# ziyu0425/PDE-Solver

Hardware: NVIDIA B200
Metric: GDOF/s (higher is better)
Workload: dtype f64

## Files before the change

### pde_solver_b200/csrc/heat2.cu

```cuda
#include <cuda.h>

#include <cmath>

#include "device.cuh"
#include "tma.cuh"

namespace {

#ifndef H_RR_STAGES
#define H_RR_STAGES 3
#endif
template <bool RR>
struct HS { static constexpr int N = RR ? H_RR_STAGES : 4; };

template <int CW, int YSB>
struct HG {
  static constexpr int TX = CW - 2, YSA = YSB + 1, TY = 2 * YSB, RA = TY + 2;
  static constexpr int BX = TX + 4, BYX = TY + 4, BYB = TY + 2;
  static constexpr int XBOX = BX * BYX, BBOX = BX * BYB;
  static constexpr int XS = (XBOX + 15) / 16 * 16, BS = (BBOX + 15) / 16 * 16;
  static constexpr int STAGE = XS + BS;
  static constexpr int RING = RA * CW;
  static constexpr int NT = 2 * CW;
  static constexpr size_t smem(int nst) { return ((size_t)nst * STAGE + 4 * RING) * sizeof(double) + nst * sizeof(uint64_t); }
};

struct H2Coef {
  double c0, cxp, cxm, cyp, cym, czp, czm, cxyp, cxym, cxzp, cxzm, cyzp, cyzm, cdp, cdm;
};
struct H2Args {
  double* y;
  double a0, a1, k1;
  int do_reduce;
  double* yc;
  int cnn0, cnn1, cnzl, cz0, cPX;
  long long cplane;
};
struct H2Geom {
  int nn0, nn1, nzl, z0, nzg, PX;
  long long plane;
  int ntx, nty, nzc, zc;
};

template <int YS>
__device__ __forceinline__ void h2_contrib(const H2Coef& C, const double (&V)[YS + 2][3], double (&aP)[YS], double (&a0)[YS],
                                           double (&aM)[YS]) {
#pragma unroll
  for (int j = 0; j < YS; ++j) {
    const int r = j + 1;
    double t = fma(C.c0, V[r][1], a0[j]);
    t = fma(C.cxp, V[r][2], t);
    t = fma(C.cxm, V[r][0], t);
    t = fma(C.cyp, V[r + 1][1], t);
    t = fma(C.cym, V[r - 1][1], t);
    t = fma(C.cxyp, V[r + 1][2], t);
    a0[j] = fma(C.cxym, V[r - 1][0], t);
    double p = fma(C.czp, V[r][1], aP[j]);
    p = fma(C.cxzp, V[r][2], p);
    p = fma(C.cyzp, V[r + 1][1], p);
    aP[j] = fma(C.cdp, V[r + 1][2], p);
    double m = C.czm * V[r][1];
    m = fma(C.cxzm, V[r][0], m);
    m = fma(C.cyzm, V[r - 1][1], m);
    aM[j] = fma(C.cdm, V[r - 1][0], m);
  }
}

template <int CW, int YSB, bool RR>
__global__ void __launch_bounds__(2 * CW, CW == 64 ? ((RR && H_RR_STAGES == 3) ? 4 : (YSB >= 4 ? 3 : (YSB == 3 ? 4 : 5))) : 6)
k_heat_post2(const __grid_constant__ CUtensorMap tmx, const __grid_constant__ CUtensorMap tmb,
             const __grid_constant__ H2Coef C, const __grid_constant__ H2Args a, const __grid_constant__ H2Geom ge,
             ReduceBuf red, double* red_out) {
  using G = HG<CW, YSB>;
  constexpr int YSA = G::YSA;
  constexpr int H_STAGES = HS<RR>::N;
  extern __shared__ __align__(128) unsigned char smem_raw[];
  double* const stage0 = reinterpret_cast<double*>(smem_raw);
  double* const ring0 = stage0 + H_STAGES * G::STAGE;
  uint64_t* const bars = reinterpret_cast<uint64_t*>(ring0 + 4 * G::RING);

  const int t = threadIdx.x;
  const int item = blockIdx.x;
  const int itx = item % ge.ntx;
  const int ity = (item / ge.ntx) % ge.nty;
  const int izc = item / (ge.ntx * ge.nty);
  const int x0 = itx * G::TX, y0 = ity * G::TY;
  const int za = izc * ge.zc;
  const int zb = min(za + ge.zc, ge.nzl);
  const int nplanes = zb - za + 4;
  const uint32_t bar0 = smem_u32(bars);
  const uint32_t stg0 = smem_u32(stage0);
  constexpr uint32_t STAGE_BYTES = G::STAGE * 8;

  auto issue = [&](int n) {
    const uint32_t bar = bar0 + 8 * (n % H_STAGES);
    const uint32_t dst = stg0 + (n % H_STAGES) * STAGE_BYTES;
    mbar_expect_tx(bar, (uint32_t)((G::XBOX + (n >= 2 ? G::BBOX : 0)) * 8));
    tma_load_4d(dst, &tmx, x0 - 2, y0 - 2, za - 2 + n + PDE_NG, 0, bar);
    if (n >= 2) tma_load_4d(dst + G::XS * 8, &tmb, x0 - 2, y0 - 1, za - 3 + n + PDE_NG, 0, bar);
  };
  if (t == 0) {
#pragma unroll
    for (int s = 0; s < H_STAGES; ++s) mbar_init(bar0 + 8 * s, 1);
    asm volatile("fence.mbarrier_init.release.cluster;" ::: "memory");
  }
  __syncthreads();
  if (t == 0)
    for (int n = 0; n < 2 && n < nplanes; ++n) issue(n);

  const int c = t % CW;
  const int s = t / CW;
  const int ix = x0 - 1 + c;
  const int cB = min(max(c, 1), CW - 2);
  const bool xfree = ix >= 1 && ix <= ge.nn0 - 2;
  unsigned mAb = 0, mBb = 0, okB = 0;
#pragma unroll
  for (int j = 0; j < YSA; ++j) {
    const int iy = y0 - 1 + s * YSA + j;
    if (xfree && iy >= 1 && iy <= ge.nn1 - 2) mAb |= 1u << j;
  }
#pragma unroll
  for (int j = 0; j < YSB; ++j) {
    const int iy = y0 + s * YSB + j;
    const bool in = c >= 1 && c <= G::TX && ix < ge.nn0 && iy < ge.nn1;
    if (in) okB |= 1u << j;
    if (in && xfree && iy >= 1 && iy <= ge.nn1 - 2) mBb |= 1u << j;
  }
  const int offA = (s * YSA) * G::BX + c;
  const int offbA = G::XS + (s * YSA) * G::BX + c + 1;
  const int offbB = G::XS + (s * YSB + 1) * G::BX + cB + 1;
  const int offxB = (s * YSB + 2) * G::BX + cB + 1;
  const int ringA = (s * YSA) * CW + c;
  const int ringB = (s * YSB) * CW + cB - 1;
  double* yrun = a.y + ((long long)ge.PX * (y0 + s * YSB) + ix) + ge.plane * za;

  double aA[YSA], aB[YSA], aC[YSA];
  double bA_[YSB], bB_[YSB], bC_[YSB];
#pragma unroll
  for (int j = 0; j < YSA; ++j) aA[j] = aB[j] = aC[j] = 0.0;
#pragma unroll
  for (int j = 0; j < YSB; ++j) bA_[j] = bB_[j] = bC_[j] = 0.0;
  double red_by = 0.0;

  auto body = [&](int i, double (&aP)[YSA], double (&a0)[YSA], double (&aM)[YSA], double (&bP)[YSB], double (&b0)[YSB],
                  double (&bM)[YSB]) {
    const int stage = i % H_STAGES;
    const int q = za - 2 + i;
    const int pA = q - 1;
    const int pB = q - 2;
    const bool finA = i >= 2, finB = i >= 4;
    double xB0[YSB], bvB[YSB];
    if (!RR && finB) {
      const double* const sx2 = stage0 + ((i - 2) % H_STAGES) * G::STAGE + offxB;
      const double* const sb1 = stage0 + ((i - 1) % H_STAGES) * G::STAGE + offbB;
#pragma unroll
      for (int j = 0; j < YSB; ++j) { xB0[j] = sx2[j * G::BX]; bvB[j] = sb1[j * G::BX]; }
    }
    mbar_wait(bar0 + 8 * stage, (uint32_t)((i / H_STAGES) & 1));
    const double* const sx = stage0 + stage * G::STAGE;
    {
      double V[YSA + 2][3];
      const double* const sp = sx + offA;
#pragma unroll
      for (int r = 0; r < YSA + 2; ++r)
#pragma unroll
        for (int cc = 0; cc < 3; ++cc)
          V[r][cc] = ((r == 0 && cc == 2) || (r == YSA + 1 && cc == 0)) ? 0.0 : sp[r * G::BX + cc];
      h2_contrib<YSA>(C, V, aP, a0, aM);
    }
    if (finA) {
      const int gz = pA + ge.z0;
      const bool zfree = gz >= 1 && gz <= ge.nzg - 2;
      const unsigned mA = zfree ? mAb : 0u;
      double* const ds = ring0 + ((pA + 4) & 3) * G::RING + ringA;
      const double* const sb = sx + offbA;
#pragma unroll
      for (int j = 0; j < YSA; ++j) ds[j * CW] = ((mA >> j) & 1u) ? a.a0 * (sb[j * G::BX] - aP[j]) : 0.0;
    }
    __syncthreads();
    if (t == 0 && i + 2 < nplanes) issue(i + 2);
    if (!RR && finA) {
      double V[YSB + 2][3];
      const double* const rp = ring0 + ((pA + 4) & 3) * G::RING + ringB;
#pragma unroll
      for (int r = 0; r < YSB + 2; ++r)
#pragma unroll
        for (int cc = 0; cc < 3; ++cc)
          V[r][cc] = ((r == 0 && cc == 2) || (r == YSB + 1 && cc == 0)) ? 0.0 : rp[r * CW + cc];
      h2_contrib<YSB>(C, V, bP, b0, bM);
    }
    if (RR && finB) {
      const int gz = pB + ge.z0;
      const int Z = (gz >> 1) - a.cz0;
      constexpr int NCX = G::TX / 2, NCY = G::TY / 2;
      if (!(gz & 1) && Z >= 0 && Z < a.cnzl && t < NCX * NCY) {
        const int cx = t % NCX, cy = t / NCX;
        const int X = (x0 >> 1) + cx, Y = (y0 >> 1) + cy;
        if (X < a.cnn0 && Y < a.cnn1) {
          const int o = (1 + 2 * cy) * CW + 1 + 2 * cx;
          const double* const r0 = ring0 + ((pB + 4) & 3) * G::RING + o;
          const double* const rm = ring0 + ((pB + 3) & 3) * G::RING + o;
          const double* const rp = ring0 + ((pB + 5) & 3) * G::RING + o;
          const double nb = ((r0[1] + r0[-1]) + (r0[CW] + r0[-CW])) + ((r0[CW + 1] + r0[-CW - 1]) + (rp[0] + rm[0])) +
                            ((rp[1] + rm[-1]) + (rp[CW] + rm[-CW])) + (rp[CW + 1] + rm[-CW - 1]);
          const int cgz = gz >> 1;
          const bool cfree = X >= 1 && X <= a.cnn0 - 2 && Y >= 1 && Y <= a.cnn1 - 2 && cgz >= 1 && cgz <= (ge.nzg >> 1) - 1;
          a.yc[(long long)a.cPX * Y + a.cplane * Z + X] = cfree ? fma(0.5, nb, r0[0]) : 0.0;
        }
      }
    }
    if (!RR && finB) {
      const int gz = pB + ge.z0;
      const bool zfree = gz >= 1 && gz <= ge.nzg - 2;
      const unsigned mB = zfree ? mBb : 0u;
      const double* const dso = ring0 + ((pB + 4) & 3) * G::RING + ringB + CW + 1;
#pragma unroll
      for (int j = 0; j < YSB; ++j) {
        const bool m = (mB >> j) & 1u;
        const double x2 = m ? fma(a.k1, dso[j * CW], fma(-a.a1, bP[j], xB0[j])) : xB0[j];
        if ((okB >> j) & 1u) yrun[j * (long long)ge.PX] = x2;
        red_by = fma(m ? bvB[j] : 0.0, x2, red_by);
      }
      yrun += ge.plane;
    }
  };

  for (int i = 0; i < nplanes; i += 3) {
    body(i, aA, aB, aC, bB_, bC_, bA_);
    if (i + 1 < nplanes) body(i + 1, aB, aC, aA, bC_, bA_, bB_);
    if (i + 2 < nplanes) body(i + 2, aC, aA, aB, bA_, bB_, bC_);
  }
  if (a.do_reduce) {
    double v[1] = {red_by};
    block_reduce_finalize<1>(v, red, red_out);
  }
}

template <int CW, int YSB, bool RR>
int launch_t(pde_ctx* c, const Grid& g, const OpDev& op, const double* x0, const double* b, const H2Args& ha_in) {
  using G = HG<CW, YSB>;
  H2Geom ge;
  ge.nn0 = g.nn[0]; ge.nn1 = g.nn[1]; ge.nzl = g.nzl; ge.z0 = g.z0; ge.nzg = g.nzg; ge.PX = g.PX; ge.plane = g.plane;
  ge.ntx = (g.nn[0] + G::TX - 1) / G::TX;
  ge.nty = (g.nn[1] + G::TY - 1) / G::TY;
  static const int zc_env = env_int("PDE_B200_P2_ZC", 64);
  int zc = zc_env < 4 ? 4 : zc_env;
  while (zc > 8 && (long long)ge.ntx * ge.nty * ((g.nzl + zc - 1) / zc) < 6LL * c->sm_count) zc /= 2;
  ge.nzc = (g.nzl + zc - 1) / zc;
  ge.zc = (g.nzl + ge.nzc - 1) / ge.nzc;
  ge.nzc = (g.nzl + ge.zc - 1) / ge.zc;
  const long long items = (long long)ge.ntx * ge.nty * ge.nzc;
  if (items > RED_MAX_BLOCKS) return 2;
  auto kern = k_heat_post2<CW, YSB, RR>;
  static bool attr_set = false;
  if (!attr_set) {
    CUDA_OK(cudaFuncSetAttribute(kern, cudaFuncAttributeMaxDynamicSharedMemorySize, (int)G::smem(HS<RR>::N)));
    CUDA_OK(cudaFuncSetAttribute(kern, cudaFuncAttributePreferredSharedMemoryCarveout, 100));
    attr_set = true;
  }
  CUtensorMap tmx, tmb;
  PDE_OK(field_tensor_map(x0, g, 1, G::BX, G::BYX, &tmx));
  PDE_OK(field_tensor_map(b, g, 1, G::BX, G::BYB, &tmb));
  H2Coef C;
  const double* h = op.h_int;
  C.c0 = h[0]; C.cxp = h[1]; C.cxm = h[2]; C.cyp = h[3]; C.cym = h[4]; C.czp = h[5]; C.czm = h[6]; C.cxyp = h[7];
  C.cxym = h[8]; C.cxzp = h[9]; C.cxzm = h[10]; C.cyzp = h[11]; C.cyzm = h[12]; C.cdp = h[13]; C.cdm = h[14];
  kern<<<(unsigned)items, G::NT, G::smem(HS<RR>::N), c->stream>>>(tmx, tmb, C, ha_in, ge, c->red, ha_in.do_reduce ? c->scal + ha_in.do_reduce - 1 : nullptr);
  c->launches++;
  CUDA_OK(cudaGetLastError());
  return 0;
}

bool heat2_applicable(const Grid& g, const OpDev& op) {
  static const int off = env_int("PDE_B200_NO_HEAT2", 0);
  if (off) return false;
  if (g.dim != 3 || g.nk != PDE_NOFF || op.ncomp != 1 || !op.uniform_diag) return false;
  return g.nn[0] >= 32 && g.nn[1] >= 8 && g.nzl >= 8;
}

template <bool RR>
int dispatch(pde_ctx* c, const Grid& g, const OpDev& op, const double* x0, const double* b, const H2Args& ha) {
  static const int cw_env = env_int("PDE_B200_P2_CW", 0);
  static const int ysb = env_int("PDE_B200_P2_YSB", 4);
  const int cw = cw_env ? cw_env : (g.nn[0] >= 128 ? 64 : 32);
  if (cw == 64 && ysb == 3) return launch_t<64, 3, RR>(c, g, op, x0, b, ha);
  if (cw == 64) return launch_t<64, 4, RR>(c, g, op, x0, b, ha);
  return launch_t<32, 4, RR>(c, g, op, x0, b, ha);
}

}

bool post2_applicable(const Grid& g, const OpDev& op) {
  if (g.dim != 3 || g.nk != PDE_NOFF || op.ncomp != 1 || !op.uniform_diag) return false;
  if (g.nn[0] < 32 || g.nn[1] < 8 || g.nzl < 8) return false;
  return !env_int("PDE_B200_NO_HEAT2", 0) || !env_int("PDE_B200_NO_POST2", 0);
}

int launch_heat_post2(pde_ctx* c, const Grid& g, const OpDev& op, const double* x0, const double* b, double* y, double c2_0,
                      double c1_1, double c2_1, int dot_slot, bool* handled) {
  *handled = false;
  if (!heat2_applicable(g, op) || !(c2_0 * op.h_dinv_int[0] > 0.0)) return 0;
  H2Args ha{};
  ha.y = y;
  ha.a0 = c2_0 * op.h_dinv_int[0];
  ha.a1 = c2_1 * op.h_dinv_int[0];
  ha.k1 = 1.0 + c1_1 + ha.a1 / ha.a0;
  ha.do_reduce = dot_slot >= 0 ? dot_slot + 1 : 0;
  const int rc = dispatch<false>(c, g, op, x0, b, ha);
  if (rc == 0) *handled = true;
  return rc == 2 ? 0 : rc;
}

int launch_heat_resid_restrict(pde_ctx* c, const Grid& gf, const Grid& gc, const OpDev& op, const double* x, const double* b,
                               double* bcoarse, bool* handled) {
  *handled = false;
  static const int off = env_int("PDE_B200_NO_RR", 0);
  if (off || !heat2_applicable(gf, op)) return 0;
  if (gf.nc[0] != 2 * gc.nc[0] || gf.nc[1] != 2 * gc.nc[1] || gf.nc[2] != 2 * gc.nc[2] || gf.z0 != 2 * gc.z0) return 0;
  H2Args ha{};
  ha.a0 = 1.0;
  ha.yc = bcoarse;
  ha.cnn0 = gc.nn[0]; ha.cnn1 = gc.nn[1]; ha.cnzl = gc.nzl; ha.cz0 = gc.z0; ha.cPX = gc.PX; ha.cplane = gc.plane;
  const int rc = dispatch<true>(c, gf, op, x, b, ha);
  if (rc == 0) *handled = true;
  return rc == 2 ? 0 : rc;
}
```

### pde_solver_b200/csrc/kernels.cu

```cuda
#include <cstring>

#include "device.cuh"
#include "tma.cuh"

template <int NC>
struct IntCoef {
  double c[PDE_NOFF][NC * NC];
};

struct StencilDev {
  const double* x;
  const double* b;
  double* y;
  const double* xprev;
  int prev_mode;
  double bconst[3];
  double bscale, ascale, c1, c2, s0;
  int do_reduce;
  int first2;
  double* defer;
};

template <int NC, bool CHEBY>
__global__ void __launch_bounds__(128)
// ... 616 lines not shown
    return 0;
  }
#define FACE_LAUNCH(CH, FU)                                                                                      \
  DISPATCH_NC(op.ncomp, (k_face_rows<NC, CH, FU><<<blocks, FACE_NT, 0, c->stream>>>(g, bc, fs, op.coef, op.dinv, op.load, \
                                                                               sd, c->red, out)))
  if (a.cheby) {
    if (full) { FACE_LAUNCH(true, true); } else { FACE_LAUNCH(true, false); }
  } else {
    if (full) { FACE_LAUNCH(false, true); } else { FACE_LAUNCH(false, false); }
  }
#undef FACE_LAUNCH
  c->launches++;
  CUDA_OK(cudaGetLastError());
  return 0;
}

__global__ void __launch_bounds__(256)
k_cg_update_flat(double* __restrict__ x, double* __restrict__ r, const double* __restrict__ p,
                 const double* __restrict__ q, long long n, int ncomp, long long cs, const double* __restrict__ scal,
                 int s_rho, int s_pap, ReduceBuf red, double* out_rho_new) {
  const double pap = scal[s_pap], rho = scal[s_rho];
  const double alpha = pap > 0.0 ? rho / pap : 0.0;
  const long long n2 = n >> 1;
  double rr = 0.0;
  for (int cidx = 0; cidx < ncomp; ++cidx) {
    double2* x2 = reinterpret_cast<double2*>(x + cidx * cs);
    double2* r2 = reinterpret_cast<double2*>(r + cidx * cs);
    const double2* p2 = reinterpret_cast<const double2*>(p + cidx * cs);
    const double2* q2 = reinterpret_cast<const double2*>(q + cidx * cs);
    if (x == nullptr) {
      for (long long i = (long long)blockIdx.x * blockDim.x + threadIdx.x; i < n2; i += (long long)gridDim.x * blockDim.x) {
        const double2 qv = q2[i];
        double2 rv = r2[i];
        rv.x = fma(-alpha, qv.x, rv.x);
        rv.y = fma(-alpha, qv.y, rv.y);
        r2[i] = rv;
        rr = fma(rv.x, rv.x, rr);
        rr = fma(rv.y, rv.y, rr);
      }
      continue;
    }
    for (long long i = (long long)blockIdx.x * blockDim.x + threadIdx.x; i < n2; i += (long long)gridDim.x * blockDim.x) {
      const double2 pv = p2[i], qv = q2[i];
      double2 xv = x2[i], rv = r2[i];
      xv.x = fma(alpha, pv.x, xv.x);
      xv.y = fma(alpha, pv.y, xv.y);
      rv.x = fma(-alpha, qv.x, rv.x);
      rv.y = fma(-alpha, qv.y, rv.y);
      x2[i] = xv;
      r2[i] = rv;
      rr = fma(rv.x, rv.x, rr);
      rr = fma(rv.y, rv.y, rr);
    }
  }
  double v[2] = {0.0, rr};
  block_reduce_finalize<2>(v, red, out_rho_new);
}

__global__ void __launch_bounds__(256)
k_cg_pupdate_flat(double* __restrict__ p, const double* __restrict__ z, long long n, int ncomp, long long cs,
                  const double* __restrict__ scal, int s_rho, int s_rho_new, int first, double* __restrict__ x,
                  int s_pap) {
  double beta = 0.0;
  if (!first) {
    const double rho = scal[s_rho];
    beta = rho > 0.0 ? scal[s_rho_new] / rho : 0.0;
  }
  const long long n2 = n >> 1;
  if (x != nullptr && !first) {
    const double pap = scal[s_pap], rho = scal[s_rho];
    const double alpha = pap > 0.0 ? rho / pap : 0.0;
    for (int cidx = 0; cidx < ncomp; ++cidx) {
      double2* p2 = reinterpret_cast<double2*>(p + cidx * cs);
      double2* x2 = reinterpret_cast<double2*>(x + cidx * cs);
      const double2* z2 = reinterpret_cast<const double2*>(z + cidx * cs);
      for (long long i = (long long)blockIdx.x * blockDim.x + threadIdx.x; i < n2; i += (long long)gridDim.x * blockDim.x) {
        const double2 zv = z2[i];
        double2 pv = p2[i], xv = x2[i];
        xv.x = fma(alpha, pv.x, xv.x);
        xv.y = fma(alpha, pv.y, xv.y);
        pv.x = fma(beta, pv.x, zv.x);
        pv.y = fma(beta, pv.y, zv.y);
        x2[i] = xv;
        p2[i] = pv;
      }
    }
    return;
  }
  for (int cidx = 0; cidx < ncomp; ++cidx) {
    double2* p2 = reinterpret_cast<double2*>(p + cidx * cs);
    const double2* z2 = reinterpret_cast<const double2*>(z + cidx * cs);
    for (long long i = (long long)blockIdx.x * blockDim.x + threadIdx.x; i < n2; i += (long long)gridDim.x * blockDim.x) {
      const double2 zv = z2[i];
      double2 pv = first ? make_double2(0.0, 0.0) : p2[i];
      pv.x = fma(beta, pv.x, zv.x);
      pv.y = fma(beta, pv.y, zv.y);
      p2[i] = pv;
    }
  }
}

int launch_cg_update(pde_ctx* c, const Grid& g, const OpDev& op, double* x, double* r, const double* p,
                     const double* q, int slot_rho, int slot_pap, int slot_rho_new, int slot_rr, int jacobi) {
  if (slot_rr != slot_rho_new + 1) PDE_FAIL("cg_update needs adjacent (rho_new, rr) slots");
  if (!jacobi) {
    int blocks = flat_blocks(c, g.total / 2, 256 * 2);
    k_cg_update_flat<<<blocks, 256, 0, c->stream>>>(x, r, p, q, g.total, op.ncomp, g.comp_stride, c->scal, slot_rho,
                                                    slot_pap, c->red, c->scal + slot_rho_new);
    c->launches++;
    CUDA_OK(cudaGetLastError());
    return 0;
  }
  RowLaunch rl = row_launch(c, g);
  DISPATCH_NC(op.ncomp, (k_cg_update<NC><<<rl.grid, rl.block, 0, c->stream>>>(
                            g, op.dinv, x, r, p, q, c->scal, slot_rho, slot_pap, c->red, c->scal + slot_rho_new,
                            c->scal + slot_rr)));
  c->launches++;
  CUDA_OK(cudaGetLastError());
  return 0;
}

int launch_cg_pupdate(pde_ctx* c, const Grid& g, const OpDev& op, double* p, const double* r_or_z, int slot_rho,
                      int slot_rho_new, int first, int jacobi, double* x_deferred, int slot_pap) {
  if (!jacobi) {
    int blocks = flat_blocks(c, g.total / 2, 256 * 2);
    k_cg_pupdate_flat<<<blocks, 256, 0, c->stream>>>(p, r_or_z, g.total, op.ncomp, g.comp_stride, c->scal, slot_rho,
                                                     slot_rho_new, first, x_deferred, slot_pap);
    c->launches++;
    CUDA_OK(cudaGetLastError());
    return 0;
  }
  RowLaunch rl = row_launch(c, g);
  DISPATCH_NC(op.ncomp, (k_cg_pupdate<NC><<<rl.grid, rl.block, 0, c->stream>>>(
                            g, op.dinv, p, r_or_z, c->scal, slot_rho, slot_rho_new, first, jacobi)));
  c->launches++;
  CUDA_OK(cudaGetLastError());
  return 0;
}

__global__ void __launch_bounds__(256)
k_dot(const double* __restrict__ a, const double* __restrict__ b, long long n, int ncomp, long long cs,
      ReduceBuf red, double* out) {
  double s = 0.0;
  const long long n2 = n >> 1;
  for (int cidx = 0; cidx < ncomp; ++cidx) {
    const double2* a2 = reinterpret_cast<const double2*>(a + cidx * cs);
    const double2* b2 = reinterpret_cast<const double2*>(b + cidx * cs);
    for (long long i = (long long)blockIdx.x * blockDim.x + threadIdx.x; i < n2; i += (long long)gridDim.x * blockDim.x) {
      const double2 u = a2[i], w = b2[i];
      s = fma(u.x, w.x, s);
      s = fma(u.y, w.y, s);
    }
  }
  double v[1] = {s};
  block_reduce_finalize<1>(v, red, out);
}

__global__ void __launch_bounds__(256)
k_axpy(double* __restrict__ y, const double* __restrict__ x, double alpha, long long n, int ncomp, long long cs,
       int mode) {
  const long long n2 = n >> 1;
  for (int cidx = 0; cidx < ncomp; ++cidx) {
    double2* y2 = reinterpret_cast<double2*>(y + cidx * cs);
    const double2* x2 = reinterpret_cast<const double2*>(x + cidx * cs);
    for (long long i = (long long)blockIdx.x * blockDim.x + threadIdx.x; i < n2; i += (long long)gridDim.x * blockDim.x) {
      if (mode == 0) {
        double2 u = y2[i];
        const double2 w = x2[i];
        u.x = fma(alpha, w.x, u.x);
        u.y = fma(alpha, w.y, u.y);
        y2[i] = u;
      } else if (mode == 1) {
        y2[i] = x2[i];
      } else {
        y2[i] = make_double2(0.0, 0.0);
      }
    }
  }
}

__global__ void __launch_bounds__(256)
k_extrapolate(double* __restrict__ u, double* __restrict__ uold, double* __restrict__ e, long long n, int ncomp,
              long long cs) {
  const long long n2 = n >> 1;
  for (int cidx = 0; cidx < ncomp; ++cidx) {
    double2* u2 = reinterpret_cast<double2*>(u + cidx * cs);
    double2* o2 = reinterpret_cast<double2*>(uold + cidx * cs);
    double2* e2 = reinterpret_cast<double2*>(e + cidx * cs);
    for (long long i = (long long)blockIdx.x * blockDim.x + threadIdx.x; i < n2; i += (long long)gridDim.x * blockDim.x) {
      const double2 a = u2[i], b = o2[i];
      const double2 d = make_double2(a.x - b.x, a.y - b.y);
      e2[i] = d;
      o2[i] = a;
      u2[i] = make_double2(a.x + d.x, a.y + d.y);
    }
  }
}
int launch_extrapolate(pde_ctx* c, const Grid& g, int ncomp, double* u, double* uold, double* e) {
  int blocks = flat_blocks(c, g.total / 2, 256 * 4);
  k_extrapolate<<<blocks, 256, 0, c->stream>>>(u, uold, e, g.total, ncomp, g.comp_stride);
  c->launches++;
  CUDA_OK(cudaGetLastError());
  return 0;
}

int launch_dot(pde_ctx* c, const Grid& g, int ncomp, const double* a, const double* b, int slot) {
  int blocks = flat_blocks(c, g.total / 2, 256 * 4);
  k_dot<<<blocks, 256, 0, c->stream>>>(a, b, g.total, ncomp, g.comp_stride, c->red, c->scal + slot);
  c->launches++;
  CUDA_OK(cudaGetLastError());
  return 0;
}
static int launch_axpy_mode(pde_ctx* c, const Grid& g, int ncomp, double* y, const double* x, double alpha, int mode) {
  int blocks = flat_blocks(c, g.total / 2, 256 * 4);
  k_axpy<<<blocks, 256, 0, c->stream>>>(y, x, alpha, g.total, ncomp, g.comp_stride, mode);
  c->launches++;
  CUDA_OK(cudaGetLastError());
  return 0;
}
int launch_zero(pde_ctx* c, const Grid& g, int ncomp, double* a) { return launch_axpy_mode(c, g, ncomp, a, a, 0.0, 2); }
int launch_copy(pde_ctx* c, const Grid& g, int ncomp, double* dst, const double* src) {
  return launch_axpy_mode(c, g, ncomp, dst, src, 0.0, 1);
}
int launch_axpy(pde_ctx* c, const Grid& g, int ncomp, double* y, const double* x, double alpha) {
  return launch_axpy_mode(c, g, ncomp, y, x, alpha, 0);
}

template <int NC>
__global__ void __launch_bounds__(128)
k_cheby_first(const __grid_constant__ Grid g, const __grid_constant__ BcDev bc, const double* __restrict__ dinv,
              const double* b, double* x, double s) {
  const long long rows = (long long)g.nn[1] * g.nzl;
  for (long long row = (long long)blockIdx.x * blockDim.y + threadIdx.y; row < rows;
       row += (long long)gridDim.x * blockDim.y) {
    const int iy = (int)(row % g.nn[1]);
    const int lz = (int)(row / g.nn[1]);
    const int gz = lz + g.z0;
    const long long rbase = (long long)g.PX * iy + g.plane * lz;
    for (int ix = threadIdx.x; ix < g.nn[0]; ix += blockDim.x) {
      double bcv;
      const bool isdir = bc_node(g, bc, ix, iy, gz, &bcv);
      const int cls = node_class(g, ix, iy, gz);
#pragma unroll
      for (int i = 0; i < NC; ++i) {
        const long long ii = rbase + ix + i * g.comp_stride;
        x[ii] = isdir ? 0.0 : s * __ldg(dinv + cls * NC + i) * b[ii];
      }
    }
  }
}

int launch_cheby_first(pde_ctx* c, const Grid& g, const BcDev& bc, const OpDev& op, const double* b, double* x,
                       double s) {
  RowLaunch rl = row_launch(c, g);
  DISPATCH_NC(op.ncomp, (k_cheby_first<NC><<<rl.grid, rl.block, 0, c->stream>>>(g, bc, op.dinv, b, x, s)));
  c->launches++;
  CUDA_OK(cudaGetLastError());
  return 0;
}

template <int NC>
__global__ void __launch_bounds__(256)
k_restrict(const __grid_constant__ Grid gf, const __grid_constant__ Grid gc, const __grid_constant__ BcDev bcc,
           const double* __restrict__ rf, double* __restrict__ bc_out) {
  const unsigned n0 = (unsigned)gc.nn[0], n1 = (unsigned)gc.nn[1];
  const long long total = (long long)n0 * n1 * gc.nzl;
  const bool small = total < (1LL << 32);
  for (long long t = (long long)blockIdx.x * blockDim.x + threadIdx.x; t < total; t += (long long)gridDim.x * blockDim.x) {
    const unsigned row = small ? (unsigned)t / n0 : (unsigned)(t / n0);
    const int ix = (int)(t - (long long)row * n0);
    const int iy = (int)(row % n1);
    const int lz = (int)(row / n1);
    const int gz = lz + gc.z0;
    const long long cbase = (long long)gc.PX * iy + gc.plane * lz;
    const int fy = gf.nc[1] > 0 ? 2 * iy : 0;
    const int flz = (gf.nc[2] > 0 ? 2 * gz : 0) - gf.z0;
    const long long fi = (long long)gf.PX * fy + gf.plane * flz + 2 * ix;
    double bcv;
    const bool isdir = bc_node(gc, bcc, ix, iy, gz, &bcv);
#pragma unroll
    for (int i = 0; i < NC; ++i) {
      double s = 0.0;
      if (!isdir) {
        const double* rp = rf + i * gf.comp_stride;
        double nb = 0.0;
        for (int k = 1; k < gf.nk; ++k) nb += rp[fi + gf.koff[k]];
        s = rp[fi] + 0.5 * nb;
      }
      bc_out[cbase + ix + i * gc.comp_stride] = s;
    }
  }
}

int launch_restrict(pde_ctx* c, const Grid& gf, const Grid& gc, const BcDev& bcc, int ncomp, const double* rf,
                    double* bcoarse) {
  const int blocks = flat_blocks(c, (long long)gc.nn[0] * gc.nn[1] * gc.nzl, 256);
  DISPATCH_NC(ncomp, (k_restrict<NC><<<blocks, 256, 0, c->stream>>>(gf, gc, bcc, rf, bcoarse)));
  c->launches++;
  CUDA_OK(cudaGetLastError());
  return 0;
}

template <int NC>
__global__ void __launch_bounds__(256)
k_prolong_add(const __grid_constant__ Grid gf, const __grid_constant__ Grid gc, const __grid_constant__ BcDev bcf,
              const double* __restrict__ xc, double* __restrict__ xf, int ghost) {
  const int nzr = gf.nzl + 2 * ghost;
  const unsigned npair = (unsigned)(gf.nn[0] + 1) / 2;
  const long long total = (long long)gf.nn[1] * nzr * npair;
  const bool small = total < (1LL << 32);
  for (long long t = (long long)blockIdx.x * blockDim.x + threadIdx.x; t < total; t += (long long)gridDim.x * blockDim.x) {
    const unsigned row = small ? (unsigned)t / npair : (unsigned)(t / npair);
    const int k = (int)(t - (long long)row * npair);
    const int iy = (int)(row % (unsigned)gf.nn[1]);
    const int lz = (int)(row / (unsigned)gf.nn[1]) - ghost;
    const int gz = lz + gf.z0;
    if (gz < 0 || gz > gf.nzg - 1) continue;
    const int ix = 2 * k;
    double bcv;
    const bool f0 = !bc_node(gf, bcf, ix, iy, gz, &bcv);
    const bool f1 = ix + 1 < gf.nn[0] && !bc_node(gf, bcf, ix + 1, iy, gz, &bcv);
    if (!f0 && !f1) continue;
    const long long fbase = (long long)gf.PX * iy + gf.plane * lz;
    const int py = gf.nc[1] > 0 ? (iy & 1) : 0;
    const int pz = gf.nc[2] > 0 ? (gz & 1) : 0;
    const int cy = gf.nc[1] > 0 ? (iy - py) / 2 : 0;
    const int clz = (gf.nc[2] > 0 ? (gz - pz) / 2 : 0) - gc.z0;
    const long long lo = (long long)gc.PX * cy + gc.plane * clz + k;
    const long long cpy = (long long)gc.PX * py + gc.plane * pz;
#pragma unroll
    for (int i = 0; i < NC; ++i) {
      const double* cp = xc + i * gc.comp_stride;
      double2* fp = reinterpret_cast<double2*>(xf + fbase + ix + i * gf.comp_stride);
      double2 v = *fp;
      const double c0 = cp[lo];
      if (f0) v.x += 0.5 * (c0 + cp[lo + cpy]);
      if (f1) v.y += 0.5 * (c0 + cp[lo + 1 + cpy]);
      *fp = v;
    }
  }
}

int launch_prolong_add(pde_ctx* c, const Grid& gf, const Grid& gc, const BcDev& bcf, int ncomp, const double* xc,
                       double* xf, int ghost) {
  const long long total = (long long)gf.nn[1] * (gf.nzl + 2 * ghost) * ((gf.nn[0] + 1) / 2);
  if (gf.nn[1] * (long long)(gf.nzl + 2 * ghost) >= (1LL << 32)) PDE_FAIL("prolongation: too many rows");
  const int blocks = flat_blocks(c, total, 256);
  DISPATCH_NC(ncomp, (k_prolong_add<NC><<<blocks, 256, 0, c->stream>>>(gf, gc, bcf, xc, xf, ghost)));
  c->launches++;
  CUDA_OK(cudaGetLastError());
  return 0;
}

__global__ void __launch_bounds__(256)
k_dense_solve(int n, const double* __restrict__ Ainv, const long long* __restrict__ idx, const double* __restrict__ b,
              double* __restrict__ x) {
  const int warp = (blockIdx.x * blockDim.x + threadIdx.x) >> 5, lane = threadIdx.x & 31;
  if (warp >= n) return;
  double s = 0.0;
  for (int j = lane; j < n; j += 32) s = fma(Ainv[(size_t)warp * n + j], b[idx[j]], s);
#pragma unroll
  for (int o = 16; o > 0; o >>= 1) s += __shfl_down_sync(0xffffffffu, s, o);
  if (lane == 0) x[idx[warp]] = s;
}

int launch_dense_solve(pde_ctx* c, int n, const double* Ainv, const long long* idx, const double* b, double* x) {
  if (n <= 0) return 0;
  int blocks = (n * 32 + 255) / 256;
  k_dense_solve<<<blocks, 256, 0, c->stream>>>(n, Ainv, idx, b, x);
  c->launches++;
  CUDA_OK(cudaGetLastError());
  return 0;
}

__global__ void __launch_bounds__(256)
k_dense_gather(int n, const long long* __restrict__ idx, const double* __restrict__ b, double* __restrict__ bglob) {
  const int j = blockIdx.x * blockDim.x + threadIdx.x;
  if (j < n) bglob[j] = idx[j] >= 0 ? b[idx[j]] : 0.0;
}
__global__ void __launch_bounds__(256)
k_dense_solve_owned(int n, const double* __restrict__ Ainv, const long long* __restrict__ idx,
                    const double* __restrict__ bglob, double* __restrict__ x) {
  const int warp = (blockIdx.x * blockDim.x + threadIdx.x) >> 5, lane = threadIdx.x & 31;
  if (warp >= n || idx[warp] < 0) return;
  double s = 0.0;
  for (int j = lane; j < n; j += 32) s = fma(Ainv[(size_t)warp * n + j], bglob[j], s);
#pragma unroll
  for (int o = 16; o > 0; o >>= 1) s += __shfl_down_sync(0xffffffffu, s, o);
  if (lane == 0) x[idx[warp]] = s;
}
int launch_dense_gather(pde_ctx* c, int n, const long long* idx, const double* b, double* bglob) {
  if (n <= 0) return 0;
  k_dense_gather<<<(n + 255) / 256, 256, 0, c->stream>>>(n, idx, b, bglob);
  c->launches++;
  CUDA_OK(cudaGetLastError());
  return 0;
}
int launch_dense_solve_owned(pde_ctx* c, int n, const double* Ainv, const long long* idx, const double* bglob,
                             double* x) {
  if (n <= 0) return 0;
  k_dense_solve_owned<<<(n * 32 + 255) / 256, 256, 0, c->stream>>>(n, Ainv, idx, bglob, x);
  c->launches++;
  CUDA_OK(cudaGetLastError());
  return 0;
}

__global__ void __launch_bounds__(128)
k_fill_ic(const __grid_constant__ Grid g, const __grid_constant__ BcDev bc, double* __restrict__ u, double value,
          int fill, int apply_bc) {
  const long long rows = (long long)g.nn[1] * g.nzl;
  for (long long row = (long long)blockIdx.x * blockDim.y + threadIdx.y; row < rows;
       row += (long long)gridDim.x * blockDim.y) {
    const int iy = (int)(row % g.nn[1]);
    const int lz = (int)(row / g.nn[1]);
    const long long rbase = (long long)g.PX * iy + g.plane * lz;
    for (int ix = threadIdx.x; ix < g.nn[0]; ix += blockDim.x) {
      double bcv;
      const bool isdir = apply_bc && bc_node(g, bc, ix, iy, lz + g.z0, &bcv);
      if (isdir) u[rbase + ix] = bcv;
      else if (fill) u[rbase + ix] = value;
    }
  }
}
__global__ void __launch_bounds__(128)
k_fill_pattern(const __grid_constant__ Grid g, const __grid_constant__ BcDev bc, int ncomp, double* __restrict__ x) {
  const long long rows = (long long)g.nn[1] * g.nzl;
  for (long long row = (long long)blockIdx.x * blockDim.y + threadIdx.y; row < rows;
       row += (long long)gridDim.x * blockDim.y) {
    const int iy = (int)(row % g.nn[1]);
    const int lz = (int)(row / g.nn[1]);
    for (int ix = threadIdx.x; ix < g.nn[0]; ix += blockDim.x) {
      double bcv;
      const bool isdir = bc_node(g, bc, ix, iy, lz + g.z0, &bcv);
      const long long node = ((long long)(lz + g.z0) * g.nn[1] + iy) * g.nn[0] + ix;
      for (int i = 0; i < ncomp; ++i)
        x[(long long)g.PX * iy + g.plane * lz + ix + i * g.comp_stride] =
            isdir ? 0.0 : sin(0.37 * (double)(node % 1000003) + i) + 0.5;
    }
  }
}
int launch_fill_pattern(pde_ctx* c, const Grid& g, const BcDev& bc, int ncomp, double* x) {
  RowLaunch rl = row_launch(c, g);
  k_fill_pattern<<<rl.grid, rl.block, 0, c->stream>>>(g, bc, ncomp, x);
  c->launches++;
  CUDA_OK(cudaGetLastError());
  return 0;
}

__global__ void __launch_bounds__(128)
k_halo_verify(const __grid_constant__ Grid g, int ncomp, int depth, const double* __restrict__ x, double scale,
              unsigned long long* bad) {
  const long long rows = (long long)g.nn[1] * 2 * depth;
  unsigned long long nbad = 0;
  for (long long row = (long long)blockIdx.x * blockDim.y + threadIdx.y; row < rows;
       row += (long long)gridDim.x * blockDim.y) {
    const int iy = (int)(row % g.nn[1]);
    const int q = (int)(row / g.nn[1]);
    const int lz = q < depth ? -1 - q : g.nzl + (q - depth);
    const int gz = lz + g.z0;
    if (gz < 0 || gz > g.nzg - 1) continue;
    for (int ix = threadIdx.x; ix < g.nn[0]; ix += blockDim.x) {
      const long long node = ((long long)gz * g.nn[1] + iy) * g.nn[0] + ix;
      for (int i = 0; i < ncomp; ++i) {
        const double want = scale * (sin(0.37 * (double)(node % 1000003) + i) + 0.5);
        if (x[(long long)g.PX * iy + g.plane * lz + ix + i * g.comp_stride] != want) ++nbad;
      }
    }
  }
  if (nbad) atomicAdd(bad, nbad);
}
int launch_halo_verify(pde_ctx* c, const Grid& g, int ncomp, int depth, const double* x, double scale,
                       unsigned long long* bad) {
  RowLaunch rl = row_launch(c, g);
  k_halo_verify<<<rl.grid, rl.block, 0, c->stream>>>(g, ncomp, depth, x, scale, bad);
  c->launches++;
  CUDA_OK(cudaGetLastError());
  return 0;
}

int launch_fill_ic(pde_ctx* c, const Grid& g, const BcDev& bc, double* u, double value, int apply_bc) {
  RowLaunch rl = row_launch(c, g);
  k_fill_ic<<<rl.grid, rl.block, 0, c->stream>>>(g, bc, u, value, 1, apply_bc);
  c->launches++;
  CUDA_OK(cudaGetLastError());
  return 0;
}
int launch_apply_bc_values(pde_ctx* c, const Grid& g, const BcDev& bc, double* u) {
  RowLaunch rl = row_launch(c, g);
  k_fill_ic<<<rl.grid, rl.block, 0, c->stream>>>(g, bc, u, 0.0, 0, 1);
  c->launches++;
  CUDA_OK(cudaGetLastError());
  return 0;
}

template <bool PACK>
__global__ void __launch_bounds__(128)
k_pack(const __grid_constant__ Grid g, int ncomp, double* __restrict__ padded, double* __restrict__ dense,
       int interleave) {
  const long long rows = (long long)g.nn[1] * g.nzl;
  const long long nloc = (long long)g.nn[0] * rows;
  for (long long row = (long long)blockIdx.x * blockDim.y + threadIdx.y; row < rows;
       row += (long long)gridDim.x * blockDim.y) {
    const int iy = (int)(row % g.nn[1]);
    const int lz = (int)(row / g.nn[1]);
    const long long rbase = (long long)g.PX * iy + g.plane * lz;
    for (int ix = threadIdx.x; ix < g.nn[0]; ix += blockDim.x) {
      const long long node = row * g.nn[0] + ix;
      for (int i = 0; i < ncomp; ++i) {
        const long long di = interleave ? node * ncomp + i : i * nloc + node;
        if (PACK) dense[di] = padded[rbase + ix + i * g.comp_stride];
        else padded[rbase + ix + i * g.comp_stride] = dense[di];
      }
    }
  }
}
int launch_pack(pde_ctx* c, const Grid& g, int ncomp, const double* padded, double* dense, int interleave) {
  RowLaunch rl = row_launch(c, g);
  k_pack<true><<<rl.grid, rl.block, 0, c->stream>>>(g, ncomp, const_cast<double*>(padded), dense, interleave);
  c->launches++;
  CUDA_OK(cudaGetLastError());
  return 0;
}
int launch_unpack(pde_ctx* c, const Grid& g, int ncomp, const double* dense, double* padded, int interleave) {
  RowLaunch rl = row_launch(c, g);
  k_pack<false><<<rl.grid, rl.block, 0, c->stream>>>(g, ncomp, padded, const_cast<double*>(dense), interleave);
  c->launches++;
  CUDA_OK(cudaGetLastError());
  return 0;
}

template <int NC>
__global__ void __launch_bounds__(128)
k_cell_rhs(const __grid_constant__ Grid g, const __grid_constant__ SimplexGeom sg, const double* __restrict__ u,
           double* __restrict__ rhs, int mode, double lam, double mu, double Emod) {
  const int axm[3] = {0, g.dim == 2 ? 2 : 1, 2};
  const long long rows = (long long)g.nn[1] * g.nzl;
  const double w = sg.vol / (double)(g.dim + 1);
  for (long long row = (long long)blockIdx.x * blockDim.y + threadIdx.y; row < rows;
       row += (long long)gridDim.x * blockDim.y) {
    const int iy = (int)(row % g.nn[1]);
    const int lz = (int)(row / g.nn[1]);
    const int gz = lz + g.z0;
    const long long rbase = (long long)g.PX * iy + g.plane * lz;
    for (int ix = threadIdx.x; ix < g.nn[0]; ix += blockDim.x) {
      const long long idx = rbase + ix;
      double acc = 0.0;
      for (int o = 0; o < 8; ++o) {
        const int ox = o & 1, oy = (o >> 1) & 1, oz = (o >> 2) & 1;
        if ((ox && (g.nc[0] == 0 || ix == 0)) || (!ox && g.nc[0] > 0 && ix == g.nn[0] - 1)) continue;
        if ((oy && (g.nc[1] == 0 || iy == 0)) || (!oy && g.nc[1] > 0 && iy == g.nn[1] - 1)) continue;
        if ((oz && (g.nc[2] == 0 || gz == 0)) || (!oz && g.nc[2] > 0 && gz == g.nzg - 1)) continue;
        const long long cell0 = idx - ox - (long long)g.PX * oy - g.plane * oz;
        for (int t = 0; t < sg.nsimp; ++t) {
          bool has = false;
          for (int a = 0; a < sg.nv; ++a) has |= (sg.corner[t][a] == o);
          if (!has) continue;
          double gu[NC][3];
#pragma unroll
          for (int i = 0; i < NC; ++i) gu[i][0] = gu[i][1] = gu[i][2] = 0.0;
          for (int a = 0; a < sg.nv; ++a) {
            const int cb = sg.corner[t][a];
            const long long vi = cell0 + (cb & 1) + (long long)g.PX * ((cb >> 1) & 1) + g.plane * ((cb >> 2) & 1);
#pragma unroll
            for (int i = 0; i < NC; ++i) {
              const double uv = u[vi + i * g.comp_stride];
              gu[i][0] = fma(uv, sg.G[t][a][0], gu[i][0]);
              gu[i][1] = fma(uv, sg.G[t][a][1], gu[i][1]);
              gu[i][2] = fma(uv, sg.G[t][a][2], gu[i][2]);
            }
          }
          double val;
          if (mode >= 2) {
            val = gu[0][0] * (mode == 3 ? Emod : 1.0);
          } else {
            double eps[NC][NC];
            double tr = 0.0;
#pragma unroll
            for (int i = 0; i < NC; ++i) {
#pragma unroll
              for (int j = 0; j < NC; ++j) eps[i][j] = 0.5 * (gu[i][axm[j]] + gu[j][axm[i]]);
              tr += eps[i][i];
            }
            double ss = 0.0;
            if (mode == 1) {
#pragma unroll
              for (int i = 0; i < NC; ++i)
#pragma unroll
                for (int j = 0; j < NC; ++j) {
                  const double dv = eps[i][j] - (i == j ? (1.0 / 3.0) * tr : 0.0);
                  ss = fma(dv, dv, ss);
                }
              val = sqrt(2.0 / 3.0 * ss);
            } else {
              double trs = 0.0;
              double sig[NC][NC];
#pragma unroll
              for (int i = 0; i < NC; ++i) {
#pragma unroll
                for (int j = 0; j < NC; ++j) sig[i][j] = 2.0 * mu * eps[i][j] + (i == j ? lam * tr : 0.0);
                trs += sig[i][i];
              }
#pragma unroll
              for (int i = 0; i < NC; ++i)
#pragma unroll
                for (int j = 0; j < NC; ++j) {
                  const double dv = sig[i][j] - (i == j ? (1.0 / 3.0) * trs : 0.0);
                  ss = fma(dv, dv, ss);
                }
              val = sqrt(3.0 / 2.0 * ss);
            }
          }
          acc = fma(val, w, acc);
        }
      }
      rhs[idx] = acc;
    }
  }
}

__device__ __forceinline__ double vm_value(const double (&gu)[3][3], int mode, double lam, double mu) {
  double eps[3][3];
  double tr = 0.0;
#pragma unroll
  for (int i = 0; i < 3; ++i) {
#pragma unroll
    for (int j = 0; j < 3; ++j) eps[i][j] = 0.5 * (gu[i][j] + gu[j][i]);
    tr += eps[i][i];
  }
  double ss = 0.0;
  if (mode == 1) {
#pragma unroll
    for (int i = 0; i < 3; ++i)
#pragma unroll
      for (int j = 0; j < 3; ++j) {
        const double dv = eps[i][j] - (i == j ? (1.0 / 3.0) * tr : 0.0);
        ss = fma(dv, dv, ss);
      }
    return sqrt(2.0 / 3.0 * ss);
  }
  double trs = 0.0, sig[3][3];
#pragma unroll
// ... 340 lines not shown
```

Before: 2.561.

## Carry heat2 stage values in registers, de-interleave RR ring, unroll prolongation

In the non-RR heat2 path, the x and b values needed two planes later are now kept in rotating registers captured from the stencil window and the defect write. They are no longer re-read from older shared-memory stages, and the defect is no longer re-read from the ring. In the RR path, ring columns are stored even/odd de-interleaved so the coarse restriction reads are less bank-conflicted. The prolongation kernel is unrolled 4x for scalar components, with raised launch bounds, to get more memory loads in flight, at the cost of extra register pressure.

```diff
diff --git a/pde_solver_b200/csrc/heat2.cu b/pde_solver_b200/csrc/heat2.cu
--- a/pde_solver_b200/csrc/heat2.cu
+++ b/pde_solver_b200/csrc/heat2.cu
@@ -128,9 +128,7 @@
   }
   const int offA = (s * YSA) * G::BX + c;
   const int offbA = G::XS + (s * YSA) * G::BX + c + 1;
-  const int offbB = G::XS + (s * YSB + 1) * G::BX + cB + 1;
-  const int offxB = (s * YSB + 2) * G::BX + cB + 1;
-  const int ringA = (s * YSA) * CW + c;
+  const int ringA = (s * YSA) * CW + (RR ? (c & 1) * (CW / 2) + (c >> 1) : c);
   const int ringB = (s * YSB) * CW + cB - 1;
   double* yrun = a.y + ((long long)ge.PX * (y0 + s * YSB) + ix) + ge.plane * za;
 
@@ -141,6 +139,9 @@
 #pragma unroll
   for (int j = 0; j < YSB; ++j) bA_[j] = bB_[j] = bC_[j] = 0.0;
   double red_by = 0.0;
+  double xo1[YSB], xo2[YSB], bo1[YSB], do1[YSB];
+#pragma unroll
+  for (int j = 0; j < YSB; ++j) xo1[j] = xo2[j] = bo1[j] = do1[j] = 0.0;
 
   auto body = [&](int i, double (&aP)[YSA], double (&a0)[YSA], double (&aM)[YSA], double (&bP)[YSB], double (&b0)[YSB],
                   double (&bM)[YSB]) {
@@ -149,13 +150,7 @@
     const int pA = q - 1;
     const int pB = q - 2;
     const bool finA = i >= 2, finB = i >= 4;
-    double xB0[YSB], bvB[YSB];
-    if (!RR && finB) {
-      const double* const sx2 = stage0 + ((i - 2) % H_STAGES) * G::STAGE + offxB;
-      const double* const sb1 = stage0 + ((i - 1) % H_STAGES) * G::STAGE + offbB;
-#pragma unroll
-      for (int j = 0; j < YSB; ++j) { xB0[j] = sx2[j * G::BX]; bvB[j] = sb1[j * G::BX]; }
-    }
+    double xq[YSB], bq[YSB] = {}, dq[YSB] = {};
     mbar_wait(bar0 + 8 * stage, (uint32_t)((i / H_STAGES) & 1));
     const double* const sx = stage0 + stage * G::STAGE;
     {
@@ -166,6 +161,10 @@
 #pragma unroll
         for (int cc = 0; cc < 3; ++cc)
           V[r][cc] = ((r == 0 && cc == 2) || (r == YSA + 1 && cc == 0)) ? 0.0 : sp[r * G::BX + cc];
+      if (!RR) {
+#pragma unroll
+        for (int j = 0; j < YSB; ++j) xq[j] = s ? V[j + 1][1] : V[j + 2][1];
+      }
       h2_contrib<YSA>(C, V, aP, a0, aM);
     }
     if (finA) {
@@ -174,8 +173,20 @@
       const unsigned mA = zfree ? mAb : 0u;
       double* const ds = ring0 + ((pA + 4) & 3) * G::RING + ringA;
       const double* const sb = sx + offbA;
-#pragma unroll
-      for (int j = 0; j < YSA; ++j) ds[j * CW] = ((mA >> j) & 1u) ? a.a0 * (sb[j * G::BX] - aP[j]) : 0.0;
+      double bA[YSA], dA[YSA];
+#pragma unroll
+      for (int j = 0; j < YSA; ++j) {
+        bA[j] = sb[j * G::BX];
+        dA[j] = ((mA >> j) & 1u) ? a.a0 * (bA[j] - aP[j]) : 0.0;
+        ds[j * CW] = dA[j];
+      }
+      if (!RR) {
+#pragma unroll
+        for (int j = 0; j < YSB; ++j) {
+          bq[j] = s ? bA[j] : bA[j + 1];
+          dq[j] = s ? dA[j] : dA[j + 1];
+        }
+      }
     }
     __syncthreads();
     if (t == 0 && i + 2 < nplanes) issue(i + 2);
@@ -192,20 +203,22 @@
     if (RR && finB) {
       const int gz = pB + ge.z0;
       const int Z = (gz >> 1) - a.cz0;
-      constexpr int NCX = G::TX / 2, NCY = G::TY / 2;
-      if (!(gz & 1) && Z >= 0 && Z < a.cnzl && t < NCX * NCY) {
-        const int cx = t % NCX, cy = t / NCX;
+      constexpr int NCX = G::TX / 2, NCY = G::TY / 2, NCXP = CW / 2;
+      static_assert(NCXP * NCY <= G::NT, "one thread per coarse node of the tile");
+      const int cx = t % NCXP, cy = t / NCXP;
+      if (!(gz & 1) && Z >= 0 && Z < a.cnzl && cx < NCX && cy < NCY) {
         const int X = (x0 >> 1) + cx, Y = (y0 >> 1) + cy;
         if (X < a.cnn0 && Y < a.cnn1) {
-          const int o = (1 + 2 * cy) * CW + 1 + 2 * cx;
-          const double* const r0 = ring0 + ((pB + 4) & 3) * G::RING + o;
-          const double* const rm = ring0 + ((pB + 3) & 3) * G::RING + o;
-          const double* const rp = ring0 + ((pB + 5) & 3) * G::RING + o;
-          const double nb = ((r0[1] + r0[-1]) + (r0[CW] + r0[-CW])) + ((r0[CW + 1] + r0[-CW - 1]) + (rp[0] + rm[0])) +
-                            ((rp[1] + rm[-1]) + (rp[CW] + rm[-CW])) + (rp[CW + 1] + rm[-CW - 1]);
+          const int e = (1 + 2 * cy) * CW + cx, o = e + CW / 2;
+          const double* const r0 = ring0 + ((pB + 4) & 3) * G::RING;
+          const double* const rm = ring0 + ((pB + 3) & 3) * G::RING;
+          const double* const rp = ring0 + ((pB + 5) & 3) * G::RING;
+          const double nb = ((r0[e + 1] + r0[e]) + (r0[o + CW] + r0[o - CW])) +
+                            ((r0[e + CW + 1] + r0[e - CW]) + (rp[o] + rm[o])) +
+                            ((rp[e + 1] + rm[e]) + (rp[o + CW] + rm[o - CW])) + (rp[e + CW + 1] + rm[e - CW]);
           const int cgz = gz >> 1;
           const bool cfree = X >= 1 && X <= a.cnn0 - 2 && Y >= 1 && Y <= a.cnn1 - 2 && cgz >= 1 && cgz <= (ge.nzg >> 1) - 1;
-          a.yc[(long long)a.cPX * Y + a.cplane * Z + X] = cfree ? fma(0.5, nb, r0[0]) : 0.0;
+          a.yc[(long long)a.cPX * Y + a.cplane * Z + X] = cfree ? fma(0.5, nb, r0[o]) : 0.0;
         }
       }
     }
@@ -213,15 +226,23 @@
       const int gz = pB + ge.z0;
       const bool zfree = gz >= 1 && gz <= ge.nzg - 2;
       const unsigned mB = zfree ? mBb : 0u;
-      const double* const dso = ring0 + ((pB + 4) & 3) * G::RING + ringB + CW + 1;
 #pragma unroll
       for (int j = 0; j < YSB; ++j) {
         const bool m = (mB >> j) & 1u;
-        const double x2 = m ? fma(a.k1, dso[j * CW], fma(-a.a1, bP[j], xB0[j])) : xB0[j];
+        const double x2 = m ? fma(a.k1, do1[j], fma(-a.a1, bP[j], xo2[j])) : xo2[j];
         if ((okB >> j) & 1u) yrun[j * (long long)ge.PX] = x2;
-        red_by = fma(m ? bvB[j] : 0.0, x2, red_by);
+        red_by = fma(m ? bo1[j] : 0.0, x2, red_by);
       }
       yrun += ge.plane;
+    }
+    if (!RR) {
+#pragma unroll
+      for (int j = 0; j < YSB; ++j) {
+        xo2[j] = xo1[j];
+        xo1[j] = xq[j];
+        bo1[j] = bq[j];
+        do1[j] = dq[j];
+      }
     }
   };
 
diff --git a/pde_solver_b200/csrc/kernels.cu b/pde_solver_b200/csrc/kernels.cu
--- a/pde_solver_b200/csrc/kernels.cu
+++ b/pde_solver_b200/csrc/kernels.cu
@@ -942,41 +942,63 @@
 }
 
 template <int NC>
-__global__ void __launch_bounds__(256)
+__global__ void __launch_bounds__(256, NC == 1 ? 3 : 8)
 k_prolong_add(const __grid_constant__ Grid gf, const __grid_constant__ Grid gc, const __grid_constant__ BcDev bcf,
               const double* __restrict__ xc, double* __restrict__ xf, int ghost) {
+  constexpr int U = NC == 1 ? 4 : 1;
   const int nzr = gf.nzl + 2 * ghost;
   const unsigned npair = (unsigned)(gf.nn[0] + 1) / 2;
   const long long total = (long long)gf.nn[1] * nzr * npair;
   const bool small = total < (1LL << 32);
-  for (long long t = (long long)blockIdx.x * blockDim.x + threadIdx.x; t < total; t += (long long)gridDim.x * blockDim.x) {
-    const unsigned row = small ? (unsigned)t / npair : (unsigned)(t / npair);
-    const int k = (int)(t - (long long)row * npair);
-    const int iy = (int)(row % (unsigned)gf.nn[1]);
-    const int lz = (int)(row / (unsigned)gf.nn[1]) - ghost;
-    const int gz = lz + gf.z0;
-    if (gz < 0 || gz > gf.nzg - 1) continue;
-    const int ix = 2 * k;
-    double bcv;
-    const bool f0 = !bc_node(gf, bcf, ix, iy, gz, &bcv);
-    const bool f1 = ix + 1 < gf.nn[0] && !bc_node(gf, bcf, ix + 1, iy, gz, &bcv);
-    if (!f0 && !f1) continue;
-    const long long fbase = (long long)gf.PX * iy + gf.plane * lz;
-    const int py = gf.nc[1] > 0 ? (iy & 1) : 0;
-    const int pz = gf.nc[2] > 0 ? (gz & 1) : 0;
-    const int cy = gf.nc[1] > 0 ? (iy - py) / 2 : 0;
-    const int clz = (gf.nc[2] > 0 ? (gz - pz) / 2 : 0) - gc.z0;
-    const long long lo = (long long)gc.PX * cy + gc.plane * clz + k;
-    const long long cpy = (long long)gc.PX * py + gc.plane * pz;
+  const long long stride = (long long)gridDim.x * blockDim.x;
+  for (long long t0 = (long long)blockIdx.x * blockDim.x + threadIdx.x; t0 < total; t0 += U * stride) {
+    bool ok[U], f0[U], f1[U];
+    long long fo[U], lo[U], cpy[U];
+#pragma unroll
+    for (int u = 0; u < U; ++u) {
+      const long long t = t0 + u * stride;
+      ok[u] = f0[u] = f1[u] = false;
+      fo[u] = lo[u] = cpy[u] = 0;
+      if (t >= total) continue;
+      const unsigned row = small ? (unsigned)t / npair : (unsigned)(t / npair);
+      const int k = (int)(t - (long long)row * npair);
+      const int iy = (int)(row % (unsigned)gf.nn[1]);
+      const int lz = (int)(row / (unsigned)gf.nn[1]) - ghost;
+      const int gz = lz + gf.z0;
+      if (gz < 0 || gz > gf.nzg - 1) continue;
+      const int ix = 2 * k;
+      double bcv;
+      f0[u] = !bc_node(gf, bcf, ix, iy, gz, &bcv);
+      f1[u] = ix + 1 < gf.nn[0] && !bc_node(gf, bcf, ix + 1, iy, gz, &bcv);
+      ok[u] = f0[u] || f1[u];
+      fo[u] = (long long)gf.PX * iy + gf.plane * lz + ix;
+      const int py = gf.nc[1] > 0 ? (iy & 1) : 0;
+      const int pz = gf.nc[2] > 0 ? (gz & 1) : 0;
+      const int cy = gf.nc[1] > 0 ? (iy - py) / 2 : 0;
+      const int clz = (gf.nc[2] > 0 ? (gz - pz) / 2 : 0) - gc.z0;
+      lo[u] = (long long)gc.PX * cy + gc.plane * clz + k;
+      cpy[u] = (long long)gc.PX * py + gc.plane * pz;
+    }
 #pragma unroll
     for (int i = 0; i < NC; ++i) {
       const double* cp = xc + i * gc.comp_stride;
-      double2* fp = reinterpret_cast<double2*>(xf + fbase + ix + i * gf.comp_stride);
-      double2 v = *fp;
-      const double c0 = cp[lo];
-      if (f0) v.x += 0.5 * (c0 + cp[lo + cpy]);
-      if (f1) v.y += 0.5 * (c0 + cp[lo + 1 + cpy]);
-      *fp = v;
+      double2 v[U];
+      double c0[U], cx0[U], cx1[U];
+#pragma unroll
+      for (int u = 0; u < U; ++u) {
+        if (!ok[u]) continue;
+        v[u] = *reinterpret_cast<const double2*>(xf + fo[u] + i * gf.comp_stride);
+        c0[u] = cp[lo[u]];
+        cx0[u] = f0[u] ? cp[lo[u] + cpy[u]] : 0.0;
+        cx1[u] = f1[u] ? cp[lo[u] + 1 + cpy[u]] : 0.0;
+      }
+#pragma unroll
+      for (int u = 0; u < U; ++u) {
+        if (!ok[u]) continue;
+        if (f0[u]) v[u].x += 0.5 * (c0[u] + cx0[u]);
+        if (f1[u]) v[u].y += 0.5 * (c0[u] + cx1[u]);
+        *reinterpret_cast<double2*>(xf + fo[u] + i * gf.comp_stride) = v[u];
+      }
     }
   }
 }
```

Result: slower. 2.491, median of 6 (-2.7%).
